# byucsl/gnumap

Hardware: AMD Instinct MI355X
Metric: reads/sec (100 bp, -a 0.9) vs human ref at 1/2/4/8 MI355X; HBM GB/s vs peak (higher is better)
Workload: dtype u32 ranks + f32 scores

## Files before the change

gnumap_amd/csrc/gm_api.cpp:

```cpp
#include "gm_host.h"
#include <algorithm>
#include <cmath>
#include <cstdio>
#include <cstring>
#include <chrono>
#include <map>
#include <memory>
#include <mutex>
#include <atomic>
#include <condition_variable>
#include <deque>
#include <functional>
#include <set>
#include <thread>
#include <fcntl.h>
#include <unistd.h>

static thread_local std::string g_err;
namespace { std::mutex g_opt_mu; std::map<std::string, const char*> g_opts; }
const char* gm_opt(const char* name) {
    const char* v = nullptr; bool have = false;
    {
        std::lock_guard<std::mutex> lk(g_opt_mu);
        auto it = g_opts.find(name);
// ... 772 lines not shown
        hipStream_t ss = b->sub_streams[s];
        uint32_t small[2]; unsigned long long ctr[GMK_N];
        HIPCHK(hipMemcpyAsync(small, b->sub_small.as<uint32_t>() + (size_t)i * 16, 8, hipMemcpyDeviceToHost, ss));
        HIPCHK(hipMemcpyAsync(ctr, view[i].counters, sizeof ctr, hipMemcpyDeviceToHost, ss));
        HIPCHK(hipMemcpyAsync(shard_host.data(), view[i].shard_cnt, shard_bytes, hipMemcpyDeviceToHost, ss));
        HIPCHK(hipStreamSynchronize(ss));
        if (ctr[GMK_BAD_QUAL] && !b->fasta) { gm_set_error("Invalid Fastq Character? (negative base probability)"); return GM_E_BAD_QUAL; }
        auto tally = [&](uint64_t& total, uint32_t& mx) { total = 0; mx = 0; for (int q = 0; q < GM_NSHARD; ++q) { uint32_t c = shard_host[(size_t)q * GM_SHARD_STRIDE]; total += c; mx = std::max(mx, c); } };
        uint64_t total; uint32_t mx;
        tally(total, mx);
        if (small[1] && mx <= region) {
            size_t slots = (size_t)ctr[GMK_HEAVY_SLOTS];
            if (b->sub_gk[s].ensure(slots * 4) || b->sub_gv[s].ensure(slots * 4)) return GM_E_NOMEM;
            view[i].gtab_keys = b->sub_gk[s].as<uint32_t>(); view[i].gtab_vals = b->sub_gv[s].as<uint32_t>();
            HIPCHK(hipMemsetAsync(b->sub_gk[s].p, 0xFF, slots * 4, ss));
            HIPCHK(hipMemsetAsync(b->sub_gv[s].p, 0, slots * 4, ss));
            { KTimer t(b, GM_K_VOTE_RETRY, ss); KCHK(gmk_vote_retry(ix->dev, dp, view[i], 1, 0, small[1], ss)); }
            HIPCHK(hipMemcpyAsync(shard_host.data(), view[i].shard_cnt, shard_bytes, hipMemcpyDeviceToHost, ss));
            HIPCHK(hipStreamSynchronize(ss));
            tally(total, mx);
        }
        if (mx > region) { overflow = true; return GM_OK; }
        ncand[i] = (uint32_t)total;
        { KTimer t(b, GM_K_NW, ss); KCHK(gmk_nw(ix->dev, dp, view[i], ncand[i], (b->len_min == b->len_max && (b->fasta || !ctr[GMK_HIGH_QUAL])) ? b->len_max : 0u, gm_qual_lo(ctr), gm_qual_hi(ctr), ss)); }
        return GM_OK;
    };
    uint32_t next_finish = 0;
    for (uint32_t i = 0; i < nsb && !overflow; ++i) {
        view[i] = make_view(i);
        hipStream_t ss = b->sub_streams[i % gm_batch::NS];
        if (i < (uint32_t)gm_batch::NS) HIPCHK(hipStreamWaitEvent(ss, b->sub_ready, 0));
        HIPCHK(hipMemsetAsync(view[i].counters, 0, GMK_N * 8, ss));
        HIPCHK(hipMemsetAsync(b->sub_small.as<uint32_t>() + (size_t)i * 16, 0, 64, ss));
        HIPCHK(hipMemsetAsync(view[i].shard_cnt, 0, shard_bytes, ss));
        HIPCHK(hipMemsetAsync(view[i].rs_overflow, 0, 2 * (size_t)view[i].n, ss));
        { KTimer t(b, GM_K_PREP, ss); KCHK(gmk_prep(ix->dev, dp, view[i], ss)); }
        { KTimer t(b, GM_K_SEED, ss); KCHK(gmk_seed(ix->dev, dp, view[i], ss, b->adaptor.empty() ? nullptr : b->full_len.as<uint16_t>() + view[i].read_base)); }
        { KTimer t(b, GM_K_VOTE, ss); KCHK(gmk_vote(ix->dev, dp, view[i], 1, dense, slots_hint, ss)); }
        if (i + 1 >= (uint32_t)gm_batch::NS) { int rc = finish(next_finish++); if (rc) return rc; }
    }
    while (next_finish < nsb && !overflow) { int rc = finish(next_finish++); if (rc) return rc; }
    for (int s = 0; s < gm_batch::NS; ++s) HIPCHK(hipStreamSynchronize(b->sub_streams[s]));
    if (overflow) return 1;
    std::vector<unsigned long long> all((size_t)nsb * GMK_N);
    HIPCHK(hipMemcpy(all.data(), b->sub_counters.p, all.size() * 8, hipMemcpyDeviceToHost));
    memset(b->counters_host, 0, sizeof b->counters_host);
    for (uint32_t i = 0; i < nsb; ++i) for (int q = 0; q < GMK_N; ++q) b->counters_host[q] += all[(size_t)i * GMK_N + q];
// ... 158 lines not shown
            }
            const uint32_t nj = j - j0;
            unsigned item_bits = 1; while ((1u << item_bits) < nj) ++item_bits;
            const size_t tmp_bytes = gmk_heavy_sort_temp_bytes((size_t)acc);
            if (b->heavy_k0.ensure((size_t)acc * 8 + 64) || b->heavy_k1.ensure((size_t)acc * 8 + 64) || b->heavy_tmp.ensure(tmp_bytes + 64) ||
                b->heavy_off.ensure((size_t)nj * 8 + 64)) return GM_E_NOMEM;
            HIPCHK(hipMemcpyAsync(b->heavy_off.p, off.data(), (size_t)nj * 8, hipMemcpyHostToDevice, st));
            KCHK(gmk_heavy_chunk(ix->dev, dp, b->dev, use_full, b->heavy_list.as<uint32_t>(), j0, nj, b->heavy_off.as<unsigned long long>(),
                                 b->heavy_k0.as<unsigned long long>(), b->heavy_k1.as<unsigned long long>(), acc, b->heavy_tmp.p, tmp_bytes, item_bits, st));
            HIPCHK(hipStreamSynchronize(st));
            GM_TRACE("heavy chunk: items %u..%u of %u, %llu keys sorted", j0, j, nh, acc);
        }
        return GM_OK;
    };
    auto read_status = [&](uint64_t& total, uint32_t& mx) -> int {
        KCHK(gmk_shard_stats(b->dev, b->small.as<uint32_t>() + 4, st));
        HIPCHK(hipMemcpyAsync(hs_small, b->small.p, 64, hipMemcpyDeviceToHost, st));
        HIPCHK(hipMemcpyAsync(hs_ctr, b->counters.p, GMK_N * 8, hipMemcpyDeviceToHost, st));
        HIPCHK(hipStreamSynchronize(st));
        total = hs_small[4]; mx = hs_small[5];
        return GM_OK;
    };
    auto read_shards = read_status;
    for (int attempt = 0;; ++attempt) {
        HIPCHK(hipMemsetAsync(b->small.p, 0, 64, st));
        HIPCHK(hipMemsetAsync(b->shards.p, 0, (size_t)GM_NSHARD * GM_SHARD_STRIDE * 4, st));
        HIPCHK(hipMemsetAsync(b->rs_overflow.p, 0, 2 * (size_t)b->n, st));
        HIPCHK(hipMemsetAsync(b->counters.as<unsigned long long>() + GMK_HEAVY_SLOTS, 0, 8, st));
        HIPCHK(hipMemsetAsync(b->counters.as<unsigned long long>() + GMK_OVERFLOW_RS, 0, 8, st));
        if (b->use_fixed && use_bucket) {
            HIPCHK(hipMemsetAsync(b->fixed_cnt.p, 0, 2 * (size_t)b->n + 32, st));
            if (++b->epoch_ctr == 0) { HIPCHK(hipMemsetAsync(b->fixed_cands.p, 0, b->fixed_cands.cap, st)); b->epoch_ctr = 1; }
            b->fixed_epoch = b->epoch_ctr;
            fill_dev_batch(b);
        } else if (b->use_fixed) HIPCHK(hipMemsetAsync(b->fixed_cnt.p, 0, 2 * (size_t)b->n, st));
        if (dp.fused) {
            HIPCHK(hipMemsetAsync(b->counters.as<unsigned long long>() + GMK_KMERS, 0, 4 * 8, st));
            HIPCHK(hipMemsetAsync(b->counters.as<unsigned long long>() + GMK_OCC_BLOCKS, 0, 2 * 8, st));
        }
        {
            KTimer t(b, GM_K_VOTE, st);
            if (use_bucket && use_pair) {
                if (!pair_direct) HIPCHK(hipMemsetAsync(b->pair_fb.p, 0, (size_t)b->n + 16, st));
                HIPCHK(hipMemsetAsync(b->pair_list.p, 0, 16, st));
                KCHK(gmk_vote_pair(ix->dev, dp, b->dev, bucket_reg, pair_direct ? nullptr : b->pair_fb.as<uint8_t>(), b->pair_list.as<uint32_t>() + 4, b->pair_list.as<uint32_t>(), st));
                KCHK(gmk_vote_bucket(ix->dev, dp, b->dev, bucket_reg, b->pair_list.as<uint32_t>() + 4, b->pair_list.as<uint32_t>(), st));
// ... 1 lines not shown
            } else if (use_bucket) { KCHK(gmk_vote_bucket(ix->dev, dp, b->dev, bucket_reg, nullptr, nullptr, st)); KCHK(gmk_vote_list(ix->dev, dp, b->dev, use_full, st)); }
            else KCHK(gmk_vote(ix->dev, dp, b->dev, use_full, dense, slots_hint, st));
            KCHK(gmk_cand_gather(b->dev, st));
        }
        if (dp.fused) { rc = collect_heavy_enqueue(); if (rc) return rc; }
        uint64_t total = 0; uint32_t mx = 0;
        rc = read_status(total, mx);
        if (rc) return rc;
        memcpy(ctr, hs_ctr, sizeof ctr);
        const uint32_t small[2] = { hs_small[0], hs_small[1] };
        if (dp.fused) { rc = fetch_heavy(hs_small[3]); if (rc) return rc; }
        if (dp.dbg & 64) {
            const double ns = (double)std::max<unsigned long long>(1, ctr[GMK_DBG8]);
            if (use_bucket) fprintf(stderr, "[gm_dbg] k_vote_bucket phases (mean clock ticks of lane 0 per sampled read, %llu samples; reads that leave early do not reach the later marks): forms + codes %.0f, "
                            "records %.0f, first walk %.0f, routing %.0f, filter pass %.0f, sweeps %.0f, store %.0f\n", ctr[GMK_DBG8], ctr[GMK_DBG0] / ns, ctr[GMK_DBG1] / ns, ctr[GMK_DBG2] / ns,
                            ctr[GMK_DBG3] / ns, ctr[GMK_DBG4] / ns, ctr[GMK_DBG5] / ns, ctr[GMK_DBG6] / ns);
            else
            fprintf(stderr, "[gm_dbg] vote phases (mean cycles per sampled read x strand, %llu samples): desc %.0f, loads+window %.0f, pass1 %.0f, pass2a %.0f, scan %.0f, "
                            "filter2 %.0f, table %.0f, emit %.0f\n", ctr[GMK_DBG8], ctr[GMK_DBG0] / ns, ctr[GMK_DBG1] / ns, ctr[GMK_DBG2] / ns, ctr[GMK_DBG3] / ns, ctr[GMK_DBG4] / ns,
                    ctr[GMK_DBG5] / ns, ctr[GMK_DBG6] / ns, ctr[GMK_DBG7] / ns);
        }
        if (ctr[GMK_BAD_QUAL] && !b->fasta) { gm_set_error("Invalid Fastq Character? (negative base probability)"); return GM_E_BAD_QUAL; }
        uint32_t n_retry = small[1];
        if (n_retry && mx <= b->dev.cand_region) {
            size_t slots = (size_t)ctr[GMK_HEAVY_SLOTS];
            const size_t budget = (size_t)gm_opt_ll("GM_RETRY_BUDGET", 1ll << 28);
            if (slots <= budget) {
                if (b->gtab_keys.ensure(slots * 4) || b->gtab_vals.ensure(slots * 4)) return GM_E_NOMEM;
                fill_dev_batch(b);
                HIPCHK(hipMemsetAsync(b->gtab_keys.p, 0xFF, slots * 4, st));
                HIPCHK(hipMemsetAsync(b->gtab_vals.p, 0, slots * 4, st));
                { KTimer t(b, GM_K_VOTE_RETRY, st); KCHK(gmk_vote_retry(ix->dev, dp, b->dev, use_full, 0, n_retry, st)); }
            } else {
                std::vector<uint32_t> list(n_retry), nent((size_t)2 * b->n);
                HIPCHK(hipMemcpyAsync(list.data(), b->retry_list.p, (size_t)n_retry * 4, hipMemcpyDeviceToHost, st));
                HIPCHK(hipMemcpyAsync(nent.data(), b->n_entries.p, nent.size() * 4, hipMemcpyDeviceToHost, st));
                HIPCHK(hipStreamSynchronize(st));
                if (b->gtab_keys.ensure(budget * 4) || b->gtab_vals.ensure(budget * 4)) return GM_E_NOMEM;
                fill_dev_batch(b);
                std::vector<unsigned long long> off(n_retry);
                KTimer t(b, GM_K_VOTE_RETRY, st);
                for (uint32_t j = 0; j < n_retry;) {
                    const uint32_t j0 = j;
                    size_t acc = 0;
                    while (j < n_retry) {
                        size_t need = 2 * (size_t)nent[list[j]], sz = 1024;
// ... 17 lines not shown
            rc = run_heavy();
            if (rc) return rc;
            rc = read_shards(total, mx);
            if (rc) return rc;
        }
        if (mx > b->dev.cand_region) {
            if (attempt > 8) { gm_set_error("candidate list keeps overflowing"); return GM_E_NOMEM; }
            size_t want = ((size_t)mx + mx / 4 + 64) * GM_NSHARD;
            if (want > 0x7FFFFFFFu) { gm_set_error("more than 2^31 candidates in one batch; map the block in smaller pieces (or use -h)"); return GM_E_BATCH_TOO_LARGE; }
            b->cand_cap = (uint32_t)want;
            if (b->cands.ensure((size_t)b->cand_cap * sizeof(GmCand))) return GM_E_NOMEM;
            fill_dev_batch(b);
            continue;
        }
        b->n_cands = (uint32_t)total;
        GM_TRACE("vote done: %llu candidates (attempt %d)", (unsigned long long)total, attempt);
        break;
    }
    if (b->raw_cap < b->n_cands + 16ull) b->raw_cap = b->n_cands + 16ull;
    if (b->raw_hits.ensure(b->raw_cap * sizeof(GmRawHit))) return GM_E_NOMEM;
    fill_dev_batch(b);
    const uint32_t nw_rows_len = (b->len_min == b->len_max && (b->fasta || ctr[GMK_HIGH_QUAL] == 0)) ? b->len_max : 0u;
    b->path += std::string(" nw=") + gmk_nw_form(dp, b->dev, b->n_cands, nw_rows_len, gm_qual_lo(ctr), gm_qual_hi(ctr));
    { KTimer t(b, GM_K_NW, st); KCHK(gmk_nw(ix->dev, dp, b->dev, b->n_cands, nw_rows_len, gm_qual_lo(ctr), gm_qual_hi(ctr), st)); }
    { KTimer t(b, GM_K_COMPACT, st); KCHK(gmk_compact(b->dev, st)); }
    if (gm_trace_on()) { HIPCHK(hipStreamSynchronize(st)); GM_TRACE("NW + compaction done"); }
    b->mapped = true;
    return GM_OK;
}

extern "C" int gm_batch_counters(gm_batch* b, gm_counters* o) {
    if (!b || !o) return GM_E_ARG;
    HIPCHK(hipSetDevice(b->ix->device));
    unsigned long long c[GMK_N];
    if (b->counters_on_host) memcpy(c, b->counters_host, sizeof c);
    else HIPCHK(hipMemcpy(c, b->counters.p, sizeof c, hipMemcpyDeviceToHost));
    memset(o, 0, sizeof *o);
    o->reads = b->n; o->kmers_searched = c[GMK_KMERS]; o->occ_calls = c[GMK_OCC]; o->occ_blocks = c[GMK_OCC_BLOCKS];
    o->seeds_used = c[GMK_SEEDS]; o->sa_hits = c[GMK_SA_HITS];
    o->lf_steps = c[GMK_LF_STEPS]; o->candidates = b->n_cands; o->nw_cells = c[GMK_NW_CELLS]; o->accepted = c[GMK_ACCEPTED];
    o->vote_retries = c[GMK_OVERFLOW_RS]; o->table_lookups = c[GMK_TAB_LOOKUPS];
    return GM_OK;
}

extern "C" const char* gm_batch_path(gm_batch* b) { return b ? b->path.c_str() : ""; }

extern "C" const char* gm_kernel_name(int which) {
// ... 693 lines not shown

extern "C" int gm_dev_nw_score(gm_index* ix, const gm_params* p, const gm_reads* reads, const uint32_t* read_idx, const uint8_t* strand,
                               const uint64_t* pos, uint32_t n, float* score, uint8_t* valid) {
    if (!ix || !p || !reads || !read_idx || !strand || !pos || !score || !p->finalized) return GM_E_ARG;
    if (ix->host_only) return GM_E_NO_DEVICE;
    HIPCHK(hipSetDevice(ix->device));
    gm_batch* b; GmDevParams dp;
    int rc = unit_batch(ix, p, reads, &b, dp, true);
    if (rc) return rc;
    std::vector<GmCand> c(n);
    for (uint32_t i = 0; i < n; ++i) {
        if (read_idx[i] >= reads->n || pos[i] > 0xFFFFFFFFull) { gm_batch_destroy(b); return GM_E_ARG; }
        c[i].rs = read_idx[i] * 2 + (strand[i] ? 1 : 0); c[i].b = (uint32_t)pos[i]; c[i].step = 0; c[i].flags = 0; c[i].pad = 0; c[i].score = 0;
    }
    do {
        b->cand_cap = std::max<uint32_t>(b->cand_cap, n + 16);
        if (b->cands.ensure((size_t)b->cand_cap * sizeof(GmCand))) { rc = GM_E_NOMEM; break; }
        fill_dev_batch(b);
        b->dev.cand_region = b->cand_cap;
        if (n && hipMemcpy(b->cands.p, c.data(), (size_t)n * sizeof(GmCand), hipMemcpyHostToDevice) != hipSuccess) { rc = GM_E_HIP; break; }
        if (hipMemset(b->shards.p, 0, (size_t)GM_NSHARD * GM_SHARD_STRIDE * 4) != hipSuccess) { rc = GM_E_HIP; break; }
        if (hipMemcpy(b->shards.p, &n, 4, hipMemcpyHostToDevice) != hipSuccess) { rc = GM_E_HIP; break; }
        uint32_t rows_len = (b->len_min == b->len_max) ? b->len_max : 0u;
        for (size_t q = 0; q < (size_t)reads->n * reads->stride && rows_len && !b->fasta; ++q) if (reads->quals[q] >= 128) rows_len = 0;
        uint32_t qlo = 255, qhi = 0;
        for (uint32_t r = 0; r < reads->n && !b->fasta; ++r)
            for (uint32_t i = 0; i < reads->len[r] && i < reads->stride; ++i) { const uint32_t qc = reads->quals[(size_t)r * reads->stride + i]; qlo = std::min(qlo, qc); qhi = std::max(qhi, qc); }
        GM_TRACE("dev_nw_score: %u probes, nw=%s", n, gmk_nw_form(dp, b->dev, n, rows_len, qlo, qhi));
        if (gmk_nw(ix->dev, dp, b->dev, n, rows_len, qlo, qhi, nullptr)) { rc = GM_E_HIP; break; }
        if (n && hipMemcpy(c.data(), b->cands.p, (size_t)n * sizeof(GmCand), hipMemcpyDeviceToHost) != hipSuccess) { rc = GM_E_HIP; break; }
    } while (0);
    gm_batch_destroy(b);
    if (rc) { gm_set_error("gm_dev_nw_score: HIP failure"); return rc; }
    for (uint32_t i = 0; i < n; ++i) { score[i] = c[i].score; if (valid) valid[i] = (c[i].flags & GMC_VALID) ? 1 : 0; }
    return GM_OK;
}

extern "C" int gm_dev_traceback(gm_index* ix, const gm_params* p, const gm_reads* reads, const uint32_t* read_idx, const uint8_t* strand,
                                const uint64_t* pos, uint32_t n, char* ops, uint32_t ops_stride, uint16_t* ops_len) {
    if (!ix || !p || !reads || !read_idx || !strand || !pos || !ops || !ops_len || !p->finalized) return GM_E_ARG;
    if (ix->host_only) return GM_E_NO_DEVICE;
    HIPCHK(hipSetDevice(ix->device));
    gm_batch* b; GmDevParams dp;
    int rc = unit_batch(ix, p, reads, &b, dp);
    if (rc) return rc;
    std::vector<GmCand> c(n);
    for (uint32_t i = 0; i < n; ++i) {
        if (read_idx[i] >= reads->n || pos[i] > 0xFFFFFFFFull) { gm_batch_destroy(b); return GM_E_ARG; }
        c[i].rs = read_idx[i] * 2 + (strand[i] ? 1 : 0); c[i].b = (uint32_t)pos[i]; c[i].step = 0; c[i].flags = 0; c[i].pad = 0; c[i].score = 0;
    }
    const uint32_t ow = gm_ops_words(b->stride);
    std::vector<unsigned long long> packed((size_t)n * ow);
// ... 512 lines not shown
```

gnumap_amd/csrc/gm_internal.h:

```cpp
#pragma once
#include <stdint.h>
#include <stddef.h>
#include <stdlib.h>
#include <string.h>

struct GmDevIndex {
    const uint32_t* bwt;
    const uint4* occ_planes;
    uint32_t occ_nblk;
    const uint32_t* sa_samples;
    const uint32_t* full_sa;
    const uint8_t* pac;
    const uint32_t* contig_off;
    uint32_t seq_len, primary, l_pac, n_seqs;
    uint32_t sa_mask, sa_shift;
    uint32_t L2[5];
};

struct GmDevParams {
    int mer, jump, kmin, nw, fast, pos_strand, neg_strand, align_is_fraction;
    int max_gap;
    int fused;
    uint32_t heavy_min;
    uint32_t hcap;
// ... 158 lines not shown
int gmk_build_kmer_compact(const uint2* tab, uint4* ctab, int T, void* stream);
int gmk_extend_kmer_table(const GmDevIndex& ix, const uint2* prev, uint2* next, int T, void* stream);
int gmk_prep(const GmDevIndex& ix, const GmDevParams& p, const GmDevBatch& b, void* stream);
int gmk_prep_rows(const GmDevIndex& ix, const GmDevParams& p, const GmDevBatch& b, void* stream);
int gmk_seed(const GmDevIndex& ix, const GmDevParams& p, const GmDevBatch& b, void* stream, const uint16_t* full_len = nullptr);
int gmk_scan_entries(const GmDevBatch& b, void* stream);
int gmk_locate_sampled(const GmDevIndex& ix, const GmDevBatch& b, unsigned long long n_entries , void* stream);
int gmk_vote(const GmDevIndex& ix, const GmDevParams& p, const GmDevBatch& b, int use_full_sa, int dense, int slots_hint, void* stream);
int gmk_cand_gather(const GmDevBatch& b, void* stream);
int gmk_shard_stats(const GmDevBatch& b, uint32_t* out , void* stream);
int gmk_build_bucket(const uint2* tab, const uint32_t* full_sa, const uint8_t* pac, uint4* bucket, int T, int ctx, void* stream);
int gmk_vote_bucket(const GmDevIndex& ix, const GmDevParams& p, const GmDevBatch& b, uint32_t max_reg, const uint32_t* rlist, const uint32_t* n_rlist, void* stream);
int gmk_vote_pair(const GmDevIndex& ix, const GmDevParams& p, const GmDevBatch& b, uint32_t max_reg, uint8_t* fallback, uint32_t* list, uint32_t* n_list, void* stream);
int gmk_vote_list(const GmDevIndex& ix, const GmDevParams& p, const GmDevBatch& b, int use_full_sa, void* stream);
int gmk_heavy_collect(const GmDevBatch& b, uint32_t heavy_min, uint32_t* n_heavy, uint32_t* heavy_list , int sum_counters,
                      const uint32_t* rlist , const uint32_t* n_rlist, void* stream);
inline uint32_t gm_pack_w2(uint32_t stride) { return (stride + 15u) / 16u; }
inline uint32_t gm_pack_words(uint32_t stride) { const uint32_t w2 = gm_pack_w2(stride); return (1u + 2u * (w2 + 1u) + 3u) & ~3u; }
size_t gmk_heavy_sort_temp_bytes(size_t n_keys);
int gmk_heavy_chunk(const GmDevIndex& ix, const GmDevParams& p, const GmDevBatch& b, int use_full_sa, const uint32_t* heavy_list, uint32_t j0, uint32_t nj,
                    const unsigned long long* key_off, unsigned long long* keys0, unsigned long long* keys1, unsigned long long n_keys, void* tmp,
                    size_t tmp_bytes, unsigned item_bits, void* stream);
int gmk_vote_retry(const GmDevIndex& ix, const GmDevParams& p, const GmDevBatch& b, int use_full_sa, uint32_t j0, uint32_t n_retry, void* stream);
int gmk_nw(const GmDevIndex& ix, const GmDevParams& p, const GmDevBatch& b, uint32_t n_cands, uint32_t rows_len, uint32_t qual_lo, uint32_t qual_hi, void* stream);
const char* gmk_nw_form(const GmDevParams& p, const GmDevBatch& b, uint32_t n_cands, uint32_t rows_len, uint32_t qual_lo, uint32_t qual_hi);
int gmk_nw_rows(const GmDevIndex& ix, const GmDevParams& p, const GmDevBatch& b, uint32_t n_cands, uint32_t L, uint32_t qual_lo, uint32_t qual_hi, void* stream);
bool gmk_nw_rows_pairs(const GmDevBatch& b, uint32_t L, uint32_t qual_lo, uint32_t qual_hi);
inline uint32_t gm_qual_lo(const unsigned long long* ctr) { return 255u - (uint32_t)ctr[GMK_QUAL_MIN]; }
inline uint32_t gm_qual_hi(const unsigned long long* ctr) { return (uint32_t)ctr[GMK_QUAL_MAX]; }
int gmk_nw_band(const GmDevIndex& ix, const GmDevParams& p, const GmDevBatch& b, uint32_t n_cands, int G, void* stream);
int gmk_traceback_band(const GmDevIndex& ix, const GmDevParams& p, const GmDevBatch& b, const GmCand* items, uint32_t n, unsigned long long* ops,
                       uint32_t ops_words, uint16_t* ops_len, const uint8_t* emit, uint32_t* cig_cnt, uint32_t* max_span, int G, void* stream);
inline uint64_t gm_band_moves_words(uint32_t n, uint32_t stride) {
    const uint64_t rows = (uint64_t)stride + 1, cap = (512ull << 20) / 8, all = (uint64_t)n * rows;
    return all < cap ? all : (cap > 128 * rows ? cap : 128 * rows);
}
size_t gmk_pair_hmm_cells(uint32_t Lmax);
int gmk_pair_hmm(const GmDevIndex& ix, const GmDevParams& p, const GmDevBatch& b, const GmCand* items, uint32_t n, double* scratch, uint32_t Lmax, float* hmm, void* stream);
int gmk_snp_deposit(float* cov, float* nuc, uint64_t bins, uint32_t bin_size, const GmDevBatch& b, const GmDevMatch* matches, const GmDevPos* positions,
                    uint32_t m0, uint32_t count, const float* post, const float* hmm, uint32_t Lmax, void* stream);
uint32_t gmk_snp_call_groups(uint64_t n);
int gmk_snp_call(const float* cov, const float* nuc, uint64_t bins, const GmDevIndex& ix, uint64_t lo, uint64_t n, float snp_pval, int monop, uint8_t* code, double* pval,
                 uint32_t* ycnt, void* stream);
int gmk_snp_gather(const float* cov, const float* nuc, uint64_t bins, const GmDevIndex& ix, uint64_t lo, uint64_t n, const uint8_t* code, const double* pval,
                   const uint32_t* ycnt, unsigned long long* off, unsigned long long base, unsigned long long cap, GmDevSnpRec* out, void* stream);
int gmk_snp_stat(const float* counts, uint32_t n, int monop, double* pval, int8_t* pos1, int8_t* pos2, uint8_t* dip, void* stream);
uint32_t gmk_track_tiles(uint64_t n);
int gmk_track_sizes(const GmDevTrack& t, void* stream);
int gmk_track_rows(const GmDevTrack& t, void* stream);
// ... 32 lines not shown
```

gnumap_amd/csrc/gm_kernels.hip:

```cpp
#include <hip/hip_runtime.h>
#include <type_traits>
#include <algorithm>
#include <atomic>
#include <cstdlib>
#include <cstring>
#include "gm_internal.h"
#include "gm_device.h"


__global__ void __launch_bounds__(256) k_expand_full_sa(GmDevIndex ix, uint32_t* full_sa, uint32_t n_sa) {
    uint32_t s = blockIdx.x * blockDim.x + threadIdx.x;
    if (s >= n_sa) return;
    uint32_t k = s << ix.sa_shift;
    if (k > ix.seq_len) return;
    uint32_t v = (s == 0) ? ix.seq_len : ix.sa_samples[s];
    full_sa[k] = v;
    for (uint32_t it = 0; it < GM_WALK_CAP; ++it) {
        k = gm_inv_psi(ix, k);
        --v;
        if ((k & ix.sa_mask) == 0) break;
        full_sa[k] = v;
    }
}

// ... 3094 lines not shown

int gmk_vote_retry(const GmDevIndex& ix, const GmDevParams& p, const GmDevBatch& b, int use_full_sa, uint32_t j0, uint32_t n_retry, void* stream) {
    if (n_retry == 0) return 0;
    hipLaunchKernelGGL(k_vote_retry, dim3(n_retry), dim3(256), 0, S_(stream), ix, p, b, use_full_sa, j0, n_retry);
    return (int)hipGetLastError();
}

static inline uint32_t lp_of(uint32_t stride) { return (stride + 7u) & ~7u; }

static bool nw_rows_ok(const GmDevParams& p, const GmDevBatch& b, uint32_t rows_len) {
    return p.max_gap == 3 && p.nw && !gm_opt_is("GM_NW", "wave") && !gm_opt_is("GM_NW", "lane") && rows_len >= 24 && rows_len <= 152 && rows_len <= b.stride;
}
const char* gmk_nw_form(const GmDevParams& p, const GmDevBatch& b, uint32_t n_cands, uint32_t rows_len, uint32_t qual_lo, uint32_t qual_hi) {
    if (p.max_gap != 3) return "k_nw_band";
    if (nw_rows_ok(p, b, rows_len)) return gmk_nw_rows_pairs(b, rows_len, qual_lo, qual_hi) ? "k_nw_rows/pairs" : "k_nw_rows/cells";
    if (gm_opt_is("GM_NW", "wave")) return "k_nw";
    const int rows_in_regs = (int)gm_opt_ll("GM_NW_ROWS", 1);
    const bool sparse = rows_in_regs && n_cands < 2.5 * b.n;
    if (sparse && b.stride <= 104) return rows_in_regs == 2 ? "k_nw_lane<13,lds>" : "k_nw_lane<13>";
    if (sparse && b.stride <= 152) return rows_in_regs == 2 ? "k_nw_lane<19,lds>" : "k_nw_lane<19>";
    return "k_nw_lane<0>";
}

int gmk_nw(const GmDevIndex& ix, const GmDevParams& p, const GmDevBatch& b, uint32_t n_cands, uint32_t rows_len, uint32_t qual_lo, uint32_t qual_hi, void* stream) {
    if (b.n == 0) return 0;
    if (p.max_gap != 3) return gmk_nw_band(ix, p, b, n_cands, p.max_gap, stream);
    const bool wave_form = gm_opt_is("GM_NW", "wave");
    if (wave_form && b.fasta) return (int)hipErrorInvalidValue;
    if (nw_rows_ok(p, b, rows_len)) return gmk_nw_rows(ix, p, b, n_cands, rows_len, qual_lo, qual_hi, stream);
    if (!wave_form) {
        const uint32_t nw_fixed = (uint32_t)gm_opt_ll("GM_NW_GRID", 0);
        uint32_t nw_grid = nw_fixed ? nw_fixed : std::min<uint32_t>(16384u, std::max<uint32_t>(2048u, n_cands / 1024u));
        const int rows_in_regs = (int)gm_opt_ll("GM_NW_ROWS", 1);
        const bool sparse = rows_in_regs && n_cands < 2.5 * b.n;
        bool big_lds = true;
        if (rows_in_regs == 2) {
            static std::atomic<unsigned long long> lds_set{ 0 };
            int dev = 0;
            if (hipGetDevice(&dev) != hipSuccess || dev < 0 || dev > 63) dev = 0;
            if (!((lds_set.load() >> dev) & 1ull)) {
                big_lds = hipFuncSetAttribute(reinterpret_cast<const void*>(&k_nw_lane<13, true>), hipFuncAttributeMaxDynamicSharedMemorySize, 2 * 13 * 256 * 8) == hipSuccess &&
                          hipFuncSetAttribute(reinterpret_cast<const void*>(&k_nw_lane<19, true>), hipFuncAttributeMaxDynamicSharedMemorySize, 2 * 19 * 256 * 8) == hipSuccess;
                if (big_lds) lds_set.fetch_or(1ull << dev);
            }
        }
        if (!big_lds && rows_in_regs == 2) return (int)hipErrorInvalidValue;
        if (sparse && rows_in_regs == 2 && b.stride <= 104) hipLaunchKernelGGL((k_nw_lane<13, true>), dim3(nw_grid), dim3(256), (size_t)2 * 13 * 256 * 8, S_(stream), ix, p, b);
        else if (sparse && rows_in_regs == 2 && b.stride <= 152) hipLaunchKernelGGL((k_nw_lane<19, true>), dim3(nw_grid), dim3(256), (size_t)2 * 19 * 256 * 8, S_(stream), ix, p, b);
        else if (sparse && b.stride <= 104) hipLaunchKernelGGL((k_nw_lane<13, false>), dim3(nw_grid), dim3(256), 0, S_(stream), ix, p, b);
        else if (sparse && b.stride <= 152) hipLaunchKernelGGL((k_nw_lane<19, false>), dim3(nw_grid), dim3(256), 0, S_(stream), ix, p, b);
        else hipLaunchKernelGGL((k_nw_lane<0, false>), dim3(nw_grid), dim3(256), 0, S_(stream), ix, p, b);
        return (int)hipGetLastError();
// ... 91 lines not shown
```

gnumap_amd/csrc/gm_nw.hip:

```cpp
#include <hip/hip_runtime.h>
#include "gm_device.h"

static inline hipStream_t S_(void* s) { return reinterpret_cast<hipStream_t>(s); }

#define GM_NWR_NCOFF 1024u
#define GM_NWR_QSTRIDE 144u
#define GM_NWR_TAB_BYTES (128u * GM_NWR_QSTRIDE)
#define GM_NWR_PAIR_SKEW 8u

template <int NCH, bool PAIRS, bool FA>
__global__ void __launch_bounds__(256, NCH <= 13 ? 4 : 3) k_nw_rows(GmDevIndex ix, GmDevParams p, GmDevBatch b, const uint32_t L, const uint32_t ntab,
                                                                    const uint32_t qlo, const uint32_t nq, const uint32_t rs) {
    constexpr uint32_t ncls = FA ? 16u : 5u;
    constexpr int NHW = (8 * NCH + 3) / 16 + 1;
    extern __shared__ __attribute__((aligned(16))) unsigned char s_tab[];
    __shared__ std::conditional_t<PAIRS, uint32_t, uint16_t> s_cls[2][2][256];
    const uint32_t qstride = PAIRS ? ncls * rs : GM_NWR_QSTRIDE, tabb = PAIRS ? nq * qstride : GM_NWR_TAB_BYTES;
    __shared__ uint32_t s_coff[GM_NWR_NCOFF];
    __shared__ uint32_t s_pre[GM_NSHARD + 4];
    {
        float sg[4][4];
#pragma unroll
        for (int g = 0; g < 4; ++g)
#pragma unroll
            for (int k = 0; k < 4; ++k) sg[g][k] = p.S256[(size_t)("acgt"[g]) * 4 + k];
        if (PAIRS) {
            for (uint32_t e = threadIdx.x; e < ntab * nq * ncls * 16u; e += 256) {
                const uint32_t n = e & 15u, rec = e >> 4, tq = rec / ncls, code = rec - ncls * tq;
                const uint32_t tab = tq / nq, qi = tq - tab * nq;
                const uint32_t mask = FA ? code : gm_code_mask(code);
                const float2 pq = FA ? p.lut[GM_LUT_FASTA + mask] : p.lut[tab * 256u + qlo + qi];
                float v[4];
#pragma unroll
                for (int g = 0; g < 4; ++g) v[g] = gm_get_val_mask(mask, pq.x, pq.y, sg[g]);
                const uint32_t x = n >> 2, y = n & 3u;
                const float2 o = make_float2(x == 0 ? v[0] : x == 1 ? v[1] : x == 2 ? v[2] : v[3], y == 0 ? v[0] : y == 1 ? v[1] : y == 2 ? v[2] : v[3]);
                *reinterpret_cast<float2*>(s_tab + tab * tabb + qi * qstride + code * rs + 8u * n) = o;
// ... 18 lines not shown
                *reinterpret_cast<float4*>(s_tab + tab * GM_NWR_TAB_BYTES + q * GM_NWR_QSTRIDE + cl * 16u) = v;
            }
        }
        const uint32_t ch = threadIdx.x, code = gm_nt4(ch);
#pragma unroll
        for (uint32_t tab = 0; tab < 2; ++tab)
#pragma unroll
            for (uint32_t st = 0; st < 2; ++st) {
                const uint32_t cl = FA ? gm_row_mask(1u, ch, st) : (code < 4u && st) ? 3u - code : code;
                const uint32_t tb = (tab < ntab ? tab : 0u) * tabb;
                s_cls[tab][st][ch] = PAIRS ? tb + cl * rs - qlo * qstride : tb + cl * 16u;
            }
    }
    const bool lds_coff = ix.n_seqs + 1 <= GM_NWR_NCOFF;
    if (lds_coff) for (uint32_t q = threadIdx.x; q <= ix.n_seqs; q += 256) s_coff[q] = ix.contig_off[q];
    const uint32_t* coff = lds_coff ? s_coff : ix.contig_off;
    const uint32_t n_cands = gm_cand_prefix(b, s_pre);
    const float gap = p.gap, gap4 = __fmul_rn(p.gap, 4.0f);
    const float ninf_gap = __fadd_rn(GM_NEG_INF, gap);
    const uint32_t* pac32 = reinterpret_cast<const uint32_t*>(ix.pac);
    const int Li = (int)L;
    const int nchunk = (Li + 7) >> 3;
    const uint32_t sh = (uint32_t)(8 * nchunk - Li);
    unsigned long long cells = 0, accepted = 0;
    for (uint32_t wi = blockIdx.x * 256 + threadIdx.x; wi < n_cands; wi += gridDim.x * 256) {
        const size_t ci = gm_cand_slot(b, s_pre, wi);
        GmCand c = b.cands[ci];
        const uint32_t r = c.rs >> 1, strand = c.rs & 1;
        if ((c.flags & 4) && b.rs_overflow[c.rs]) continue;
        const bool ok = gm_window_ok(ix, coff, c.b, L);
        float result = 0.0f;
        if (ok && p.nw) {
            uint2 XB[NCH], XQ[NCH];
            {
                const uint8_t* rb = b.bases + (size_t)r * b.stride;
                const uint8_t* rq = b.quals + (size_t)r * b.stride;
                const uint32_t selx = strand ? 0x03020100u : 0x04050607u, sely = strand ? 0x07060504u : 0x00010203u;
#pragma unroll
                for (int k = 0; k < NCH; ++k) {
                    XB[k] = make_uint2(0u, 0u); XQ[k] = make_uint2(0u, 0u);
                    if (k < nchunk) {
                        const int fo = Li - 8 - 8 * k;
                        const uint32_t off = strand ? (uint32_t)(8 * k) : (uint32_t)(fo > 0 ? fo : 0);
                        uint2 tb, tq = make_uint2(0u, 0u);
                        __builtin_memcpy(&tb, rb + off, 8);
                        if (!FA) __builtin_memcpy(&tq, rq + off, 8);
                        uint2 ob = make_uint2(__builtin_amdgcn_perm(tb.y, tb.x, selx), __builtin_amdgcn_perm(tb.y, tb.x, sely));
                        uint2 oq = make_uint2(__builtin_amdgcn_perm(tq.y, tq.x, selx), __builtin_amdgcn_perm(tq.y, tq.x, sely));
                        if (k == nchunk - 1 && sh != 0u) {
                            const uint32_t s8 = strand ? 0u : 8u * sh;
                            const unsigned long long wb = (((unsigned long long)ob.y << 32) | ob.x) >> s8, wq = (((unsigned long long)oq.y << 32) | oq.x) >> s8;
                            ob = make_uint2((uint32_t)wb, (uint32_t)(wb >> 32)); oq = make_uint2((uint32_t)wq, (uint32_t)(wq >> 32));
                        }
                        XB[k] = ob; XQ[k] = oq;
                    }
                }
            }
            uint32_t HW[NHW];
            {
                const uint32_t g0 = c.b + L - 1u, n0 = g0 >> 4, s = 30u - 2u * (g0 & 15u);
                uint32_t W[NHW + 1];
#pragma unroll
                for (int j = 0; j <= NHW; ++j) {
                    const uint32_t idx = n0 >= (uint32_t)j ? n0 - (uint32_t)j : 0u;
                    const uint32_t x = pac32[idx];
                    W[j] = __builtin_amdgcn_perm(x, x, 0x00010203u);
                }
#pragma unroll
                for (int m = 0; m < NHW; ++m) HW[m] = __builtin_amdgcn_alignbit(W[m + 1], W[m], s);
            }
            const uint32_t tab = (ntab > 1u && r < b.illumina_until) ? 1u : 0u;
            const auto* const clsrow = s_cls[tab][strand];
            float P[7];
#pragma unroll
            for (int d = 0; d < 7; ++d) P[d] = d <= 3 ? __fmul_rn(gap, (float)(3 - d)) : GM_NEG_INF;
            uint32_t cc[7];
#pragma unroll
            for (int d = 0; d < 7; ++d) cc[d] = d > 3 ? 0u : PAIRS ? (((HW[0] << 2) >> (2 * (3 - d))) & 15u) << 3 : ((HW[0] >> (2 * (3 - d))) & 3u) << 2;
            auto row_vals = [&](uint32_t bword, uint32_t qword, uint32_t shift) -> uint32_t {
                const uint32_t chv = (bword >> shift) & 255u;
                const uint32_t co = clsrow[chv];
                const uint32_t qv = (qword >> shift) & 255u;
                return __umul24(qv, qstride) + co;
            };
            auto cell_val = [&](const uint32_t v, int d) -> float { return *reinterpret_cast<const float*>(s_tab + v + cc[d]); };
            auto slide = [&](uint32_t hw, uint32_t hwp, uint32_t pos) {
#pragma unroll
                for (int d = 6; d >= 1; --d) cc[d] = cc[d - 1];
                if (PAIRS) cc[0] = (uint32_t)((((unsigned long long)hw << 32) | hwp) >> (27u + pos)) & 0x78u;
                else cc[0] = ((hw >> pos) & 3u) << 2;
// ... 80 lines not shown
#pragma unroll
                for (int bb = B0; bb < 8; ++bb) co[bb] = clsrow[((bb < 4 ? bw.x : bw.y) >> ((bb & 3) << 3)) & 255u];
#pragma unroll
                for (int bb = B0; bb < 8; ++bb) {
                    const uint32_t v = __umul24(((bb < 4 ? qw.x : qw.y) >> ((bb & 3) << 3)) & 255u, qstride) + co[bb];
                    if (PAR) { if (bb < 4) row_int(v, hw_lo, hw_lo, 2u * (12u + bb)); else row_int(v, hw_hi, hw_lo, 2u * (bb - 4u)); }
                    else row_int(v, hw_lo, hw_lo, 2u * (4u + bb));
                }
            };
            if (nchunk >= 4) {
                using I0 = std::integral_constant<int, 0>; using I1 = std::integral_constant<int, 1>; using I4 = std::integral_constant<int, 4>;
                tail_rows(0, 0, 4, std::true_type{});
                rows8(0, I0{}, I4{});
                const int k_last = nchunk - 3;
                for (int k = 1; k <= k_last; ++k) { if (k & 1) rows8(k, I1{}, I0{}); else rows8(k, I0{}, I0{}); }
                for (int k = k_last + 1; k < nchunk; ++k) {
                    const int lo = 8 * k, hi = (8 * k + 8 < Li) ? 8 * k + 8 : Li, cut = Li - 4;
                    if (lo < cut) tail_rows(k, lo, hi < cut ? hi : cut, std::false_type{});
                    if (hi > cut) tail_rows(k, lo > cut ? lo : cut, hi, std::true_type{});
                }
            } else {
                for (int k = 0; k < nchunk; ++k) tail_rows(k, 8 * k, (8 * k + 8 < Li) ? 8 * k + 8 : Li, std::true_type{});
            }
            if (Li >= 7) cells += (unsigned long long)(7 * Li - 12);
            else for (int i = 0; i < Li; ++i) { int lo = i - 3 < 0 ? 0 : i - 3, hi = i + 3 >= Li ? Li - 1 : i + 3; cells += (unsigned long long)(hi - lo + 1); }
            result = P[3];
        } else if (!p.nw) {
            result = (float)c.step;
        }
        uint8_t fl = c.flags & 4;
        if (ok) {
            fl |= GMC_VALID;
            if (result > 0.0f) atomicMax(reinterpret_cast<int*>(&b.top_score[r]), __float_as_int(result));
            if ((double)result >= b.min_score[r]) {
                fl |= GMC_ACCEPT;
                atomicAdd(&b.hit_count[r], 1u);
                ++accepted;
            }
        }
        b.cands[ci].score = result;
        b.cands[ci].flags = fl;
    }
    gm_count(b, GMK_NW_CELLS, cells);
    gm_count(b, GMK_ACCEPTED, accepted);
}

static uint32_t nw_pair_rs() {
    const long long k = gm_opt_ll("GM_NW_PAIR_SKEW", GM_NWR_PAIR_SKEW);
    return 128u + ((k >= 0 && k <= 64 && k % 8 == 0) ? (uint32_t)k : GM_NWR_PAIR_SKEW);
}
static size_t nw_pair_lds(uint32_t ntab, uint32_t qlo, uint32_t qhi) {
    return (qlo <= qhi && qhi < 128u) ? (size_t)ntab * (qhi - qlo + 1u) * 5u * nw_pair_rs() : 0;
}
#define GM_NWR_FASTA_CELLS_BYTES 256u

template <bool FA>
static bool nw_pairs_fit(bool narrow, size_t lds_cells, size_t lds) {
    int per_cells = 0, per_pairs = 0;
    hipError_t e0, e1;
    if (narrow) {
        e0 = hipOccupancyMaxActiveBlocksPerMultiprocessor(&per_cells, k_nw_rows<13, false, FA>, 256, lds_cells);
        e1 = hipOccupancyMaxActiveBlocksPerMultiprocessor(&per_pairs, k_nw_rows<13, true, FA>, 256, lds);
    } else {
        e0 = hipOccupancyMaxActiveBlocksPerMultiprocessor(&per_cells, k_nw_rows<19, false, FA>, 256, lds_cells);
        e1 = hipOccupancyMaxActiveBlocksPerMultiprocessor(&per_pairs, k_nw_rows<19, true, FA>, 256, lds);
    }
    return e0 == hipSuccess && e1 == hipSuccess && per_pairs > 0 && per_pairs >= per_cells;
}

bool gmk_nw_rows_pairs(const GmDevBatch& b, uint32_t L, uint32_t qlo, uint32_t qhi) {
    if (gm_opt_is("GM_NW_CELLS", "b32")) return false;
    const uint32_t ntab = b.illumina_until ? 2u : 1u;
    const size_t lds = b.fasta ? (size_t)16u * nw_pair_rs() : nw_pair_lds(ntab, qlo, qhi);
    const size_t lds_cells = b.fasta ? (size_t)GM_NWR_FASTA_CELLS_BYTES : (size_t)ntab * GM_NWR_TAB_BYTES;
    if (!lds) return false;
    return b.fasta ? nw_pairs_fit<true>(L <= 104, lds_cells, lds) : nw_pairs_fit<false>(L <= 104, lds_cells, lds);
}

int gmk_nw_rows(const GmDevIndex& ix, const GmDevParams& p, const GmDevBatch& b, uint32_t n_cands, uint32_t L, uint32_t qlo, uint32_t qhi, void* stream) {
    if (b.n == 0) return 0;
    const uint32_t ntab = (b.illumina_until && !b.fasta) ? 2u : 1u;
    const bool pairs = gmk_nw_rows_pairs(b, L, qlo, qhi);
    const size_t lds = b.fasta ? (pairs ? (size_t)16u * nw_pair_rs() : (size_t)GM_NWR_FASTA_CELLS_BYTES) : pairs ? nw_pair_lds(ntab, qlo, qhi) : (size_t)ntab * GM_NWR_TAB_BYTES;
    const uint32_t nq = b.fasta ? 1u : pairs ? qhi - qlo + 1u : 0u, q0 = (pairs && !b.fasta) ? qlo : 0u;
    const uint32_t nw_fixed = (uint32_t)gm_opt_ll("GM_NW_GRID", 0);
    const bool narrow = L <= 104;
#define GM_NWR_LAUNCH_(N, PR, FA, FB)                                                                                                          \
    hipLaunchKernelGGL((k_nw_rows<N, PR, FA>), dim3(nw_fixed ? nw_fixed : resident_grid(k_nw_rows<N, PR, FA>, 256, lds, FB)), dim3(256), lds, \
                       S_(stream), ix, p, b, L, ntab, q0, nq, nw_pair_rs())
#define GM_NWR_LAUNCH(N, PR, FB) do { if (b.fasta) GM_NWR_LAUNCH_(N, PR, true, FB); else GM_NWR_LAUNCH_(N, PR, false, FB); } while (0)
    if (narrow && pairs) GM_NWR_LAUNCH(13, true, 1024u);
    else if (narrow) GM_NWR_LAUNCH(13, false, 1024u);
    else if (pairs) GM_NWR_LAUNCH(19, true, 768u);
    else GM_NWR_LAUNCH(19, false, 768u);
#undef GM_NWR_LAUNCH_
#undef GM_NWR_LAUNCH
    return (int)hipGetLastError();
}
```

Baseline: 1.000 billion.

## Hoist NW candidate, read and reference loads ahead of dependent work in k_nw_rows

Restructures the per-candidate prologue of k_nw_rows. The candidate record is read as one 16-byte load, and the read bases and qualities are fetched as 16-byte chunks before any dependent work, then split into 8-byte chunks with perm ops. The packed reference window is loaded as a contiguous vector block, with a register shift when it is clamped at the genome start. It also skips the rs_overflow lookup when the host reports no superseded reads, computes the band-cell count once per thread, and writes score and flags with a single 8-byte store. The aim is to cut scattered small loads and latency stalls, at the cost of more registers, which could lower occupancy.

Result: faster. 1.037 billion (median of 6 runs) (+3.7%).

```diff
diff --git a/gnumap_amd/csrc/gm_api.cpp b/gnumap_amd/csrc/gm_api.cpp
--- a/gnumap_amd/csrc/gm_api.cpp
+++ b/gnumap_amd/csrc/gm_api.cpp
@@ -818,7 +818,7 @@
         }
         if (mx > region) { overflow = true; return GM_OK; }
         ncand[i] = (uint32_t)total;
-        { KTimer t(b, GM_K_NW, ss); KCHK(gmk_nw(ix->dev, dp, view[i], ncand[i], (b->len_min == b->len_max && (b->fasta || !ctr[GMK_HIGH_QUAL])) ? b->len_max : 0u, gm_qual_lo(ctr), gm_qual_hi(ctr), ss)); }
+        { KTimer t(b, GM_K_NW, ss); KCHK(gmk_nw(ix->dev, dp, view[i], ncand[i], (b->len_min == b->len_max && (b->fasta || !ctr[GMK_HIGH_QUAL])) ? b->len_max : 0u, gm_qual_lo(ctr), gm_qual_hi(ctr), small[1] != 0, ss)); }
         return GM_OK;
     };
     uint32_t next_finish = 0;
@@ -1023,6 +1023,7 @@
         return GM_OK;
     };
     auto read_shards = read_status;
+    bool any_superseded = false;
     for (int attempt = 0;; ++attempt) {
         HIPCHK(hipMemsetAsync(b->small.p, 0, 64, st));
         HIPCHK(hipMemsetAsync(b->shards.p, 0, (size_t)GM_NSHARD * GM_SHARD_STRIDE * 4, st));
@@ -1070,6 +1071,7 @@
         }
         if (ctr[GMK_BAD_QUAL] && !b->fasta) { gm_set_error("Invalid Fastq Character? (negative base probability)"); return GM_E_BAD_QUAL; }
         uint32_t n_retry = small[1];
+        any_superseded = n_retry != 0 || !heavy.empty();
         if (n_retry && mx <= b->dev.cand_region) {
             size_t slots = (size_t)ctr[GMK_HEAVY_SLOTS];
             const size_t budget = (size_t)gm_opt_ll("GM_RETRY_BUDGET", 1ll << 28);
@@ -1133,7 +1135,7 @@
     fill_dev_batch(b);
     const uint32_t nw_rows_len = (b->len_min == b->len_max && (b->fasta || ctr[GMK_HIGH_QUAL] == 0)) ? b->len_max : 0u;
     b->path += std::string(" nw=") + gmk_nw_form(dp, b->dev, b->n_cands, nw_rows_len, gm_qual_lo(ctr), gm_qual_hi(ctr));
-    { KTimer t(b, GM_K_NW, st); KCHK(gmk_nw(ix->dev, dp, b->dev, b->n_cands, nw_rows_len, gm_qual_lo(ctr), gm_qual_hi(ctr), st)); }
+    { KTimer t(b, GM_K_NW, st); KCHK(gmk_nw(ix->dev, dp, b->dev, b->n_cands, nw_rows_len, gm_qual_lo(ctr), gm_qual_hi(ctr), any_superseded, st)); }
     { KTimer t(b, GM_K_COMPACT, st); KCHK(gmk_compact(b->dev, st)); }
     if (gm_trace_on()) { HIPCHK(hipStreamSynchronize(st)); GM_TRACE("NW + compaction done"); }
     b->mapped = true;
@@ -1873,12 +1875,12 @@
         if (hipMemset(b->shards.p, 0, (size_t)GM_NSHARD * GM_SHARD_STRIDE * 4) != hipSuccess) { rc = GM_E_HIP; break; }
         if (hipMemcpy(b->shards.p, &n, 4, hipMemcpyHostToDevice) != hipSuccess) { rc = GM_E_HIP; break; }
         uint32_t rows_len = (b->len_min == b->len_max) ? b->len_max : 0u;
-        for (size_t q = 0; q < (size_t)reads->n * reads->stride && rows_len && !b->fasta; ++q) if (reads->quals[q] >= 128) rows_len = 0;
         uint32_t qlo = 255, qhi = 0;
         for (uint32_t r = 0; r < reads->n && !b->fasta; ++r)
             for (uint32_t i = 0; i < reads->len[r] && i < reads->stride; ++i) { const uint32_t qc = reads->quals[(size_t)r * reads->stride + i]; qlo = std::min(qlo, qc); qhi = std::max(qhi, qc); }
+        if (qhi >= 128) rows_len = 0;
         GM_TRACE("dev_nw_score: %u probes, nw=%s", n, gmk_nw_form(dp, b->dev, n, rows_len, qlo, qhi));
-        if (gmk_nw(ix->dev, dp, b->dev, n, rows_len, qlo, qhi, nullptr)) { rc = GM_E_HIP; break; }
+        if (gmk_nw(ix->dev, dp, b->dev, n, rows_len, qlo, qhi, false, nullptr)) { rc = GM_E_HIP; break; }
         if (n && hipMemcpy(c.data(), b->cands.p, (size_t)n * sizeof(GmCand), hipMemcpyDeviceToHost) != hipSuccess) { rc = GM_E_HIP; break; }
     } while (0);
     gm_batch_destroy(b);
diff --git a/gnumap_amd/csrc/gm_internal.h b/gnumap_amd/csrc/gm_internal.h
--- a/gnumap_amd/csrc/gm_internal.h
+++ b/gnumap_amd/csrc/gm_internal.h
@@ -204,9 +204,9 @@
                     const unsigned long long* key_off, unsigned long long* keys0, unsigned long long* keys1, unsigned long long n_keys, void* tmp,
                     size_t tmp_bytes, unsigned item_bits, void* stream);
 int gmk_vote_retry(const GmDevIndex& ix, const GmDevParams& p, const GmDevBatch& b, int use_full_sa, uint32_t j0, uint32_t n_retry, void* stream);
-int gmk_nw(const GmDevIndex& ix, const GmDevParams& p, const GmDevBatch& b, uint32_t n_cands, uint32_t rows_len, uint32_t qual_lo, uint32_t qual_hi, void* stream);
+int gmk_nw(const GmDevIndex& ix, const GmDevParams& p, const GmDevBatch& b, uint32_t n_cands, uint32_t rows_len, uint32_t qual_lo, uint32_t qual_hi, bool any_superseded, void* stream);
 const char* gmk_nw_form(const GmDevParams& p, const GmDevBatch& b, uint32_t n_cands, uint32_t rows_len, uint32_t qual_lo, uint32_t qual_hi);
-int gmk_nw_rows(const GmDevIndex& ix, const GmDevParams& p, const GmDevBatch& b, uint32_t n_cands, uint32_t L, uint32_t qual_lo, uint32_t qual_hi, void* stream);
+int gmk_nw_rows(const GmDevIndex& ix, const GmDevParams& p, const GmDevBatch& b, uint32_t n_cands, uint32_t L, uint32_t qual_lo, uint32_t qual_hi, bool any_superseded, void* stream);
 bool gmk_nw_rows_pairs(const GmDevBatch& b, uint32_t L, uint32_t qual_lo, uint32_t qual_hi);
 inline uint32_t gm_qual_lo(const unsigned long long* ctr) { return 255u - (uint32_t)ctr[GMK_QUAL_MIN]; }
 inline uint32_t gm_qual_hi(const unsigned long long* ctr) { return (uint32_t)ctr[GMK_QUAL_MAX]; }
diff --git a/gnumap_amd/csrc/gm_kernels.hip b/gnumap_amd/csrc/gm_kernels.hip
--- a/gnumap_amd/csrc/gm_kernels.hip
+++ b/gnumap_amd/csrc/gm_kernels.hip
@@ -3140,12 +3140,12 @@
     return "k_nw_lane<0>";
 }
 
-int gmk_nw(const GmDevIndex& ix, const GmDevParams& p, const GmDevBatch& b, uint32_t n_cands, uint32_t rows_len, uint32_t qual_lo, uint32_t qual_hi, void* stream) {
+int gmk_nw(const GmDevIndex& ix, const GmDevParams& p, const GmDevBatch& b, uint32_t n_cands, uint32_t rows_len, uint32_t qual_lo, uint32_t qual_hi, bool any_superseded, void* stream) {
     if (b.n == 0) return 0;
     if (p.max_gap != 3) return gmk_nw_band(ix, p, b, n_cands, p.max_gap, stream);
     const bool wave_form = gm_opt_is("GM_NW", "wave");
     if (wave_form && b.fasta) return (int)hipErrorInvalidValue;
-    if (nw_rows_ok(p, b, rows_len)) return gmk_nw_rows(ix, p, b, n_cands, rows_len, qual_lo, qual_hi, stream);
+    if (nw_rows_ok(p, b, rows_len)) return gmk_nw_rows(ix, p, b, n_cands, rows_len, qual_lo, qual_hi, any_superseded, stream);
     if (!wave_form) {
         const uint32_t nw_fixed = (uint32_t)gm_opt_ll("GM_NW_GRID", 0);
         uint32_t nw_grid = nw_fixed ? nw_fixed : std::min<uint32_t>(16384u, std::max<uint32_t>(2048u, n_cands / 1024u));
diff --git a/gnumap_amd/csrc/gm_nw.hip b/gnumap_amd/csrc/gm_nw.hip
--- a/gnumap_amd/csrc/gm_nw.hip
+++ b/gnumap_amd/csrc/gm_nw.hip
@@ -10,9 +10,11 @@
 
 template <int NCH, bool PAIRS, bool FA>
 __global__ void __launch_bounds__(256, NCH <= 13 ? 4 : 3) k_nw_rows(GmDevIndex ix, GmDevParams p, GmDevBatch b, const uint32_t L, const uint32_t ntab,
-                                                                    const uint32_t qlo, const uint32_t nq, const uint32_t rs) {
+                                                                    const uint32_t qlo, const uint32_t nq, const uint32_t rs, const uint32_t sup) {
     constexpr uint32_t ncls = FA ? 16u : 5u;
     constexpr int NHW = (8 * NCH + 3) / 16 + 1;
+    constexpr int NP = (NCH + 1) / 2;
+    constexpr int NWL = (NHW + 4) / 4, NWW = 4 * NWL;
     extern __shared__ __attribute__((aligned(16))) unsigned char s_tab[];
     __shared__ std::conditional_t<PAIRS, uint32_t, uint16_t> s_cls[2][2][256];
     const uint32_t qstride = PAIRS ? ncls * rs : GM_NWR_QSTRIDE, tabb = PAIRS ? nq * qstride : GM_NWR_TAB_BYTES;
@@ -77,50 +79,101 @@
     const int Li = (int)L;
     const int nchunk = (Li + 7) >> 3;
     const uint32_t sh = (uint32_t)(8 * nchunk - Li);
-    unsigned long long cells = 0, accepted = 0;
+    const int m_last = (nchunk - 1) >> 1;
+    const bool odd = (nchunk & 1) != 0;
+    const int omax = (int)b.stride - 16;
+    const uint32_t nlast = (ix.l_pac - 1u) >> 4;
+    unsigned long long band_cells = 0;
+    if (Li >= 7) band_cells = (unsigned long long)(7 * Li - 12);
+    else for (int i = 0; i < Li; ++i) { int lo = i - 3 < 0 ? 0 : i - 3, hi = i + 3 >= Li ? Li - 1 : i + 3; band_cells += (unsigned long long)(hi - lo + 1); }
+    uint32_t scored = 0, accepted = 0;
     for (uint32_t wi = blockIdx.x * 256 + threadIdx.x; wi < n_cands; wi += gridDim.x * 256) {
         const size_t ci = gm_cand_slot(b, s_pre, wi);
-        GmCand c = b.cands[ci];
+        GmCand c;
+        uint32_t c_hi;
+        {
+            uint4 cw;
+            __builtin_memcpy(&cw, &b.cands[ci], 16);
+            c.rs = cw.x; c.b = cw.y; c_hi = cw.z;
+            c.step = (uint16_t)c_hi; c.flags = (uint8_t)(c_hi >> 16);
+        }
         const uint32_t r = c.rs >> 1, strand = c.rs & 1;
-        if ((c.flags & 4) && b.rs_overflow[c.rs]) continue;
+        uint4 TB[NP], TQ[NP];
+        {
+            unsigned long long row = (unsigned long long)r * b.stride;
+            asm("" : "+v"(row));
+            const uint8_t* rb = b.bases + row;
+            const uint8_t* rq = b.quals + row;
+            uint32_t fwd = strand - 1u;
+            asm("" : "+v"(fwd));
+#pragma unroll
+            for (int m = 0; m < NP; ++m) {
+                const int orv = 16 * m - ((odd && m == m_last) ? 8 : 0), ofw = Li - 16 - 16 * m;
+                const uint32_t orc = (uint32_t)(orv < omax ? orv : omax), ofc = (uint32_t)(ofw > 0 ? ofw : 0);
+                const uint32_t off = orc + (fwd & (ofc - orc));
+                __builtin_memcpy(&TB[m], rb + off, 16);
+                if (!FA) __builtin_memcpy(&TQ[m], rq + off, 16);
+                else TQ[m] = make_uint4(0u, 0u, 0u, 0u);
+            }
+        }
+        const uint32_t g0 = c.b + L - 1u, n0 = g0 >> 4;
+        const uint32_t n0c = n0 < nlast ? n0 : nlast;
+        uint32_t A[NWW];
+        {
+            const uint32_t* wp = pac32 + (n0c >= (uint32_t)(NWW - 1) ? n0c - (uint32_t)(NWW - 1) : 0u);
+#pragma unroll
+            for (int q = 0; q < NWL; ++q) {
+                uint4 t;
+                __builtin_memcpy(&t, wp + 4 * q, 16);
+                A[4 * q] = t.x; A[4 * q + 1] = t.y; A[4 * q + 2] = t.z; A[4 * q + 3] = t.w;
+            }
+        }
+        const double min_score = b.min_score[r];
+        uint32_t superseded = 0u;
+        if (sup && (c.flags & 4)) superseded = b.rs_overflow[c.rs];
         const bool ok = gm_window_ok(ix, coff, c.b, L);
+        if (superseded) continue;
         float result = 0.0f;
         if (ok && p.nw) {
             uint2 XB[NCH], XQ[NCH];
             {
-                const uint8_t* rb = b.bases + (size_t)r * b.stride;
-                const uint8_t* rq = b.quals + (size_t)r * b.stride;
-                const uint32_t selx = strand ? 0x03020100u : 0x04050607u, sely = strand ? 0x07060504u : 0x00010203u;
-#pragma unroll
-                for (int k = 0; k < NCH; ++k) {
-                    XB[k] = make_uint2(0u, 0u); XQ[k] = make_uint2(0u, 0u);
-                    if (k < nchunk) {
-                        const int fo = Li - 8 - 8 * k;
-                        const uint32_t off = strand ? (uint32_t)(8 * k) : (uint32_t)(fo > 0 ? fo : 0);
-                        uint2 tb, tq = make_uint2(0u, 0u);
-                        __builtin_memcpy(&tb, rb + off, 8);
-                        if (!FA) __builtin_memcpy(&tq, rq + off, 8);
-                        uint2 ob = make_uint2(__builtin_amdgcn_perm(tb.y, tb.x, selx), __builtin_amdgcn_perm(tb.y, tb.x, sely));
-                        uint2 oq = make_uint2(__builtin_amdgcn_perm(tq.y, tq.x, selx), __builtin_amdgcn_perm(tq.y, tq.x, sely));
-                        if (k == nchunk - 1 && sh != 0u) {
-                            const uint32_t s8 = strand ? 0u : 8u * sh;
-                            const unsigned long long wb = (((unsigned long long)ob.y << 32) | ob.x) >> s8, wq = (((unsigned long long)oq.y << 32) | oq.x) >> s8;
-                            ob = make_uint2((uint32_t)wb, (uint32_t)(wb >> 32)); oq = make_uint2((uint32_t)wq, (uint32_t)(wq >> 32));
+                const uint32_t selx = strand ? 0x03020100u : 0x04050607u;
+                const uint32_t s8 = strand ? 0u : 8u * sh;
+#pragma unroll
+                for (int m = 0; m < NP; ++m) {
+                    const uint32_t sel = m <= m_last ? selx : 0x0C0C0C0Cu;
+                    uint2 lo[2], hi[2];
+#pragma unroll
+                    for (int a = 0; a < (FA ? 1 : 2); ++a) {
+                        const uint4 t = a ? TQ[m] : TB[m];
+                        lo[a] = make_uint2(__builtin_amdgcn_perm(t.w, t.x, sel), __builtin_amdgcn_perm(t.z, t.y, sel));
+                        hi[a] = make_uint2(__builtin_amdgcn_perm(t.y, t.z, sel), __builtin_amdgcn_perm(t.x, t.w, sel));
+                        if (m == m_last && (odd || sh != 0u)) {
+                            const unsigned long long l64 = ((unsigned long long)lo[a].y << 32) | lo[a].x, h64 = ((unsigned long long)hi[a].y << 32) | hi[a].x;
+                            const unsigned long long nl = odd ? h64 >> s8 : (l64 >> s8) | ((h64 << 1) << (63u - s8)), nh = odd ? 0ull : h64 >> s8;
+                            lo[a] = make_uint2((uint32_t)nl, (uint32_t)(nl >> 32)); hi[a] = make_uint2((uint32_t)nh, (uint32_t)(nh >> 32));
                         }
-                        XB[k] = ob; XQ[k] = oq;
                     }
+                    if (FA) { lo[1] = make_uint2(0u, 0u); hi[1] = make_uint2(0u, 0u); }
+                    XB[2 * m] = lo[0]; XQ[2 * m] = lo[1];
+                    if (2 * m + 1 < NCH) { XB[2 * m + 1] = hi[0]; XQ[2 * m + 1] = hi[1]; }
                 }
             }
             uint32_t HW[NHW];
             {
-                const uint32_t g0 = c.b + L - 1u, n0 = g0 >> 4, s = 30u - 2u * (g0 & 15u);
+                if (n0c < (uint32_t)(NWW - 1)) {
+                    const uint32_t up = (uint32_t)(NWW - 1) - n0c;
+#pragma unroll
+                    for (int bit = 1; bit < NWW; bit <<= 1) {
+                        const bool mv = (up & (uint32_t)bit) != 0u;
+#pragma unroll
+                        for (int q = NWW - 1; q >= 0; --q) A[q] = mv ? A[q >= bit ? q - bit : 0] : A[q];
+                    }
+                }
+                const uint32_t s = 30u - 2u * (g0 & 15u);
                 uint32_t W[NHW + 1];
 #pragma unroll
-                for (int j = 0; j <= NHW; ++j) {
-                    const uint32_t idx = n0 >= (uint32_t)j ? n0 - (uint32_t)j : 0u;
-                    const uint32_t x = pac32[idx];
-                    W[j] = __builtin_amdgcn_perm(x, x, 0x00010203u);
-                }
+                for (int j = 0; j <= NHW; ++j) W[j] = __builtin_amdgcn_perm(A[NWW - 1 - j], A[NWW - 1 - j], 0x00010203u);
 #pragma unroll
                 for (int m = 0; m < NHW; ++m) HW[m] = __builtin_amdgcn_alignbit(W[m + 1], W[m], s);
             }
@@ -247,8 +300,7 @@
             } else {
                 for (int k = 0; k < nchunk; ++k) tail_rows(k, 8 * k, (8 * k + 8 < Li) ? 8 * k + 8 : Li, std::true_type{});
             }
-            if (Li >= 7) cells += (unsigned long long)(7 * Li - 12);
-            else for (int i = 0; i < Li; ++i) { int lo = i - 3 < 0 ? 0 : i - 3, hi = i + 3 >= Li ? Li - 1 : i + 3; cells += (unsigned long long)(hi - lo + 1); }
+            ++scored;
             result = P[3];
         } else if (!p.nw) {
             result = (float)c.step;
@@ -257,17 +309,17 @@
         if (ok) {
             fl |= GMC_VALID;
             if (result > 0.0f) atomicMax(reinterpret_cast<int*>(&b.top_score[r]), __float_as_int(result));
-            if ((double)result >= b.min_score[r]) {
+            if ((double)result >= min_score) {
                 fl |= GMC_ACCEPT;
                 atomicAdd(&b.hit_count[r], 1u);
                 ++accepted;
             }
         }
-        b.cands[ci].score = result;
-        b.cands[ci].flags = fl;
+        const uint2 out = make_uint2((c_hi & 0xFF00FFFFu) | ((uint32_t)fl << 16), __float_as_uint(result));
+        __builtin_memcpy(reinterpret_cast<unsigned char*>(&b.cands[ci]) + 8, &out, 8);
     }
-    gm_count(b, GMK_NW_CELLS, cells);
-    gm_count(b, GMK_ACCEPTED, accepted);
+    gm_count(b, GMK_NW_CELLS, (unsigned long long)scored * band_cells);
+    gm_count(b, GMK_ACCEPTED, (unsigned long long)accepted);
 }
 
 static uint32_t nw_pair_rs() {
@@ -302,7 +354,7 @@
     return b.fasta ? nw_pairs_fit<true>(L <= 104, lds_cells, lds) : nw_pairs_fit<false>(L <= 104, lds_cells, lds);
 }
 
-int gmk_nw_rows(const GmDevIndex& ix, const GmDevParams& p, const GmDevBatch& b, uint32_t n_cands, uint32_t L, uint32_t qlo, uint32_t qhi, void* stream) {
+int gmk_nw_rows(const GmDevIndex& ix, const GmDevParams& p, const GmDevBatch& b, uint32_t n_cands, uint32_t L, uint32_t qlo, uint32_t qhi, bool any_superseded, void* stream) {
     if (b.n == 0) return 0;
     const uint32_t ntab = (b.illumina_until && !b.fasta) ? 2u : 1u;
     const bool pairs = gmk_nw_rows_pairs(b, L, qlo, qhi);
@@ -312,7 +364,7 @@
     const bool narrow = L <= 104;
 #define GM_NWR_LAUNCH_(N, PR, FA, FB)                                                                                                          \
     hipLaunchKernelGGL((k_nw_rows<N, PR, FA>), dim3(nw_fixed ? nw_fixed : resident_grid(k_nw_rows<N, PR, FA>, 256, lds, FB)), dim3(256), lds, \
-                       S_(stream), ix, p, b, L, ntab, q0, nq, nw_pair_rs())
+                       S_(stream), ix, p, b, L, ntab, q0, nq, nw_pair_rs(), any_superseded ? 1u : 0u)
 #define GM_NWR_LAUNCH(N, PR, FB) do { if (b.fasta) GM_NWR_LAUNCH_(N, PR, true, FB); else GM_NWR_LAUNCH_(N, PR, false, FB); } while (0)
     if (narrow && pairs) GM_NWR_LAUNCH(13, true, 1024u);
     else if (narrow) GM_NWR_LAUNCH(13, false, 1024u);
```
